# fraunhoferhhi/vvenc

Hardware: AMD Instinct MI355X
Metric: frames/sec + bit-exact vs CPU, 1080p/4K 10-bit preset=faster at 1/2/4/8 GPU (higher is better)
Workload: dtype i16; 1 GPU; BASELINE configs[1]: hot-path work lists RECORDED from the reference encoder (1920x1080 10-bit synthetic clip, 65 frames, preset faster; one picture per temporal layer), replayed resident in HBM: a step = one picture's integer-ME SAD windows + sub-pel SATD stages + table calls + fused TU transform/quant lists + DMVR lists on 5 HIP streams; steps follow the GOP's 1:1:2:4:8:16 layer mix from the key; hip_streams=5, sample_pairs_per_frame=175309451, coefficients_per_frame=6951461, recorded_calls_outside_the_lists=0

## Files before the change

vvenc_amd/csrc/me.hip:

```cpp
#include <stdlib.h>
#ifndef VVHIP_ME_HU
#define VVHIP_ME_HU 2
#endif
#ifndef VVHIP_ME_STAGE_WAVES
#define VVHIP_ME_STAGE_WAVES 6
#endif
#ifndef VVHIP_ME_ITEM_WAVES
#define VVHIP_ME_ITEM_WAVES 8
#endif
#include <string.h>
#include <algorithm>
#include <vector>
#include "common.h"
#include "hadtile.h"

struct vvhip_me_plan
{
  int bitDepth = 0, nCands = 0, nStages = 0, nItems = 0, nMaskItems = 0, maxPlane = 0;
  int wavesInt = 0, wavesStage = 0, wavesItem = 0, wavesItemMain = 0, ldsInt = 0, ldsStage = 0;
  int intBig = 0, ldsIntSmall = 0;
  int intLarge = 0, ldsIntMid = 0;
  bool stageAtomic = false;
  bool intSplit = false;
  bool timing = false; hipEvent_t ev[5] = { nullptr, nullptr, nullptr, nullptr, nullptr };
// ... 148 lines not shown
  { 0, 64, 0, 0 }, { -1, 63, 2, 0 }, { -2, 62, 4, 0 }, { -2, 60, 7, -1 }, { -2, 58, 10, -2 }, { -3, 57, 12, -2 }, { -4, 56, 14, -2 }, { -4, 55, 15, -2 }, { -4, 54, 16, -2 },
  { -5, 53, 18, -2 }, { -6, 52, 20, -2 }, { -6, 49, 24, -3 }, { -6, 46, 28, -4 }, { -5, 44, 29, -4 }, { -4, 42, 30, -4 }, { -4, 39, 33, -4 }, { -4, 36, 36, -4 } };

static int stageTap( int frac, int k, int filterMode, int altHpel )
{
  if( altHpel && frac == 8 ) return kAltHpel[k];
  if( filterMode == 2 )
  {
    const int ph = frac << 1;
    return ( k < 2 || k > 5 ) ? 0 : ( ph <= 16 ? kChroma4[ph][k - 2] : kChroma4[32 - ph][5 - k] );
  }
  const int p = frac <= 8 ? frac : 16 - frac, kk = frac <= 8 ? k : 7 - k;
  return filterMode == 0 ? kLuma8[p][kk] : kLuma6[p][kk];
}

static std::vector<int32_t> stageTapTables( int bitDepth )
{
  const int headRoom = 14 - bitDepth > 2 ? 14 - bitDepth : 2, vScale = 1 << ( 10 - headRoom ), hScale = 1 << ( 2 + headRoom );
  std::vector<int32_t> tapTab( 6 * 192, 0 );
  for( int mode = 0; mode < 3; mode++ ) for( int alt = 0; alt < 2; alt++ )
  {
    int32_t* t = &tapTab[( mode * 2 + alt ) * 192];
    const int set = ( mode == 2 && !alt ) ? 0 : ( mode == 0 ? 2 : 1 ), k0 = set == 0 ? 2 : ( set == 1 ? 1 : 0 ), np = set == 0 ? 2 : ( set == 1 ? 3 : 4 );
    for( int f = 0; f < 16; f++ )
    {
      for( int k = 0; k < 8; k++ ) t[f * 8 + k] = stageTap( f, k, mode, alt ) * vScale;
      for( int i = 0; i < 4; i++ ) t[128 + f * 4 + i] = i < np ? ( int32_t ) ( ( ( uint32_t ) ( stageTap( f, k0 + 2 * i, mode, alt ) * hScale ) & 0xffffu ) | ( ( uint32_t ) ( stageTap( f, k0 + 2 * i + 1, mode, alt ) * hScale ) << 16 ) ) : 0;
    }
  }
  return tapTab;
}

__device__ __forceinline__ void stagePos( const vvhip_me_stage_job& j, int k, int& tx, int& ty )
{
  constexpr uint32_t RX  = 1u | 1u << 2 | 1u << 4 | 0u << 6 | 2u << 8 | 0u << 10 | 2u << 12 | 0u << 14 | 2u << 16;
  constexpr uint32_t RYH = 1u | 0u << 2 | 2u << 4 | 1u << 6 | 1u << 8 | 0u << 10 | 0u << 12 | 2u << 14 | 2u << 16;
  constexpr uint32_t RYQ = 1u | 0u << 2 | 2u << 4 | 0u << 6 | 0u << 8 | 1u << 10 | 1u << 12 | 2u << 14 | 2u << 16;
  const int rx = ( int ) ( ( RX >> ( 2 * k ) ) & 3u ) - 1, ry = ( int ) ( ( ( j.i_frac == 2 ? RYH : RYQ ) >> ( 2 * k ) ) & 3u ) - 1;
  tx = ( rx + j.base_qx ) * j.i_frac * 4; ty = ( ry + j.base_qy ) * j.i_frac * 4;
}

template<int NT> struct VTaps { int c[NT]; };
template<int K0, int K1>
__device__ __forceinline__ void loadVTaps( const int* tapL, int fyk, VTaps<K1 - K0 + 1>& vt )
{
#pragma unroll
  for( int t = 0; t < K1 - K0 + 1; t++ ) vt.c[t] = tapL[fyk * 8 + K0 + t];
}
__device__ __forceinline__ int madLo( uint32_t v, int c, int acc ) { int r; asm( "v_mad_i32_i16 %0, %1, %2, %3" : "=v"( r ) : "v"( v ), "v"( c ), "v"( acc ) ); return r; }
__device__ __forceinline__ int madHi( uint32_t v, int c, int acc ) { int r; asm( "v_mad_i32_i16 %0, %1, %2, %3 op_sel:[1,0,0,0]" : "=v"( r ) : "v"( v ), "v"( c ), "v"( acc ) ); return r; }
__device__ __forceinline__ int mulLo( uint32_t v, int c ) { int r; asm( "v_mad_i32_i16 %0, %1, %2, 0" : "=v"( r ) : "v"( v ), "v"( c ) ); return r; }
__device__ __forceinline__ int med3( int v, int hi ) { int r; asm( "v_med3_i32 %0, %1, 0, %2" : "=v"( r ) : "v"( v ), "v"( hi ) ); return r; }
__device__ __forceinline__ int mulHi( uint32_t v, int c ) { int r; asm( "v_mad_i32_i16 %0, %1, %2, 0 op_sel:[1,0,0,0]" : "=v"( r ) : "v"( v ), "v"( c ) ); return r; }
template<int K0, int K1>
__device__ __forceinline__ void predRow( const int16_t* tv , int w, int y, int syk, bool anyFrac,
                                         const VTaps<K1 - K0 + 1>& vt, int headRoom, uint32_t maxPk, uint32_t ( &o )[4] )
{
  constexpr int NT = K1 - K0 + 1;
  if( anyFrac )
  {
    int acc[8];
#pragma unroll
    for( int t = 0; t < NT; t++ )
    {
      const int c = vt.c[t];
      const u32x4 r = *reinterpret_cast<const u32x4*>( tv + __mul24( y + syk + t + 1, w ) );
      if( t == 0 )
      {
        acc[0] = mulLo( r.x, c ); acc[1] = mulHi( r.x, c ); acc[2] = mulLo( r.y, c ); acc[3] = mulHi( r.y, c );
        acc[4] = mulLo( r.z, c ); acc[5] = mulHi( r.z, c ); acc[6] = mulLo( r.w, c ); acc[7] = mulHi( r.w, c );
      }
      else
      {
        acc[0] = madLo( r.x, c, acc[0] ); acc[1] = madHi( r.x, c, acc[1] ); acc[2] = madLo( r.y, c, acc[2] ); acc[3] = madHi( r.y, c, acc[3] );
        acc[4] = madLo( r.z, c, acc[4] ); acc[5] = madHi( r.z, c, acc[5] ); acc[6] = madLo( r.w, c, acc[6] ); acc[7] = madHi( r.w, c, acc[7] );
      }
    }
    const int maxS = ( int ) ( ( ( maxPk & 0xffffu ) << 16 ) | 0xffffu );
#pragma unroll
    for( int i = 0; i < 8; i++ ) acc[i] = med3( acc[i], maxS );
#pragma unroll
    for( int i = 0; i < 4; i++ ) o[i] = __builtin_amdgcn_perm( ( uint32_t ) acc[2 * i + 1], ( uint32_t ) acc[2 * i], 0x07060302u );
  }
  else
  {
    const u32x4 r = *reinterpret_cast<const u32x4*>( tv + __mul24( y + syk + 4 - K0, w ) );
    const uint32_t rw[4] = { r.x, r.y, r.z, r.w };
    const s16x2 sh = { ( short ) headRoom, ( short ) headRoom }, z = { 0, 0 };
#pragma unroll
    for( int i = 0; i < 4; i++ )
      o[i] = __builtin_bit_cast( uint32_t, __builtin_elementwise_min( __builtin_elementwise_max( __builtin_bit_cast( s16x2, rw[i] ) >> sh, z ), __builtin_bit_cast( s16x2, maxPk ) ) );
  }
}

__device__ __forceinline__ void avgInts( const uint32_t ( &ra )[4], const uint32_t ( &rb )[4], int ( &o )[4] )
{
#pragma unroll
  for( int i = 0; i < 4; i++ ) o[i] = dot2( pkAdd( ra[i], rb[i] ), 0x00010001u, 2 ) >> 2;
}

__device__ __forceinline__ int dot2s( uint32_t a, uint32_t b, int c ) { int r; asm( "v_dot2_i32_i16 %0, %1, %2, %3" : "=v"( r ) : "v"( a ), "v"( b ), "s"( c ) ); return r; }

template<int K0, int K1, bool ONE>
__device__ __forceinline__ void firstPass( const char* refB, int rs, int nH, int G, int log2G, int rowsT, int ldsPitch, int v0, int hx0, int hx1, int hx2,
                                           const uint32_t* tapP, int16_t* tmp, int tid, int offS, int headRoom, uint32_t biasPk )
{
  constexpr int NT = K1 - K0 + 1, NP = NT / 2, B0 = ( NT - 2 ) / 2, HU = VVHIP_ME_HU;
  const int txOne = v0 == 0 ? hx0 : ( v0 == 1 ? hx1 : hx2 );
  for( int ub = tid; ub < nH; ub += HU * 64 )
  {
    u32x4 LA[HU], LB[HU]; int fxs[HU], at[HU]; bool ok[HU];
#pragma unroll
    for( int q = 0; q < HU; q++ )
    {
      const int u = ub + q * 64;
      ok[q] = u < nH;
      const int uu = ok[q] ? u : ub;
      const int x0 = ( uu & ( G - 1 ) ) << 3, rr = uu >> log2G;
      int r = rr, txv = txOne;
      if( !ONE )
      {
        const int vl = ( rr >= rowsT ) + ( rr >= 2 * rowsT ), v = v0 + vl;
        r = rr - __mul24( vl, rowsT ); txv = v == 0 ? hx0 : ( v == 1 ? hx1 : hx2 );
      }
      fxs[q] = txv & 15; at[q] = __mul24( rr, ldsPitch ) + x0;
      const uint32_t off = ( uint32_t ) ( __mul24( r, rs ) + x0 + ( txv >> 4 ) + 8 ) * 2u;
      LA[q] = ld16o( refB, fxs[q] ? off + ( uint32_t ) ( 2 * ( K0 - 3 ) ) : off );
      if( fxs[q] ) LB[q] = ld16o( refB, off + ( uint32_t ) ( 2 * ( K0 - 3 + NT - 1 ) ) );
    }
#pragma unroll
    for( int q = 0; q < HU; q++ )
    {
      if( !ok[q] ) continue;
      const int fxv = fxs[q];
      const u32x4 A = LA[q];
      u32x4 ov;
      if( fxv )
      {
        const u32x4 B = LB[q];
        uint32_t W[4 + NP], S[4 + NP];
        W[0] = A.x; W[1] = A.y; W[2] = A.z; W[3] = A.w;
        S[B0] = B.x; S[B0 + 1] = B.y; S[B0 + 2] = B.z; S[B0 + 3] = B.w;
#pragma unroll
        for( int m = B0 - 1; m >= 0; m-- ) S[m] = __builtin_amdgcn_alignbit( W[m + 1], W[m], 16 );
#pragma unroll
        for( int m = 4; m < 4 + NP - 1; m++ ) W[m] = __builtin_amdgcn_alignbit( S[m], S[m - 1], 16 );
        uint32_t cp[NP];
#pragma unroll
        for( int i = 0; i < NP; i++ ) cp[i] = tapP[fxv * 4 + i];
        uint32_t o[4];
#pragma unroll
        for( int qq = 0; qq < 4; qq++ )
        {
          int e = dot2s( W[qq], cp[0], offS ), d = dot2s( S[qq], cp[0], offS );
#pragma unroll
          for( int i = 1; i < NP; i++ ) { e = dot2( W[qq + i], cp[i], e ); d = dot2( S[qq + i], cp[i], d ); }
          o[qq] = __builtin_amdgcn_perm( ( uint32_t ) d, ( uint32_t ) e, 0x06050201u );
        }
        ov.x = o[0]; ov.y = o[1]; ov.z = o[2]; ov.w = o[3];
      }
      else
      {
        const uint32_t aw[4] = { A.x, A.y, A.z, A.w };
        const s16x2 sh = { ( short ) headRoom, ( short ) headRoom };
        uint32_t o[4];
#pragma unroll
        for( int qq = 0; qq < 4; qq++ ) o[qq] = pkAdd( __builtin_bit_cast( uint32_t, __builtin_bit_cast( s16x2, aw[qq] ) << sh ), biasPk );
        ov.x = o[0]; ov.y = o[1]; ov.z = o[2]; ov.w = o[3];
      }
      *reinterpret_cast<u32x4*>( tmp + at[q] ) = ov;
    }
  }
}

constexpr int ST_STAGE_MASK = 0x3fffff, ST_VAR_SHIFT = 22;
constexpr int ST_UNIT_CONT = 1 << 28, ST_UNIT_MORE = 1 << 29, ST_UNIT_ATOMIC = 1 << 30;

template<int K0, int K1, bool GEN>
__device__ __forceinline__ void stageBody( const MePlanes& P, const MeArgs& a, const WaveSpan span, int16_t* lds, uint32_t* pairCost, const int wv )
{
  constexpr int NT = K1 - K0 + 1;
#define ST_SYNC() { __builtin_amdgcn_fence( __ATOMIC_ACQ_REL, "wavefront" ); __builtin_amdgcn_wave_barrier(); }
  const int tid = threadIdx.x & 63, nthr = 64, lane = tid, bd = a.bitDepth;
  const int headRoom = 14 - bd > 2 ? 14 - bd : 2;
  const int offS = ( 1 << ( headRoom - 1 ) ) << 8;
  const uint32_t biasPk = ( uint32_t ) ( 1 << ( headRoom - 1 ) ) * 0x00010001u;
  const uint32_t maxPk = ( uint32_t ) ( ( 1 << bd ) - 1 ) * 0x00010001u;
  int* tapL = reinterpret_cast<int*>( lds );
  uint32_t* tapP = reinterpret_cast<uint32_t*>( lds ) + 128;
  int* posL = reinterpret_cast<int*>( lds ) + 128 + 64;
  uint32_t* costL = reinterpret_cast<uint32_t*>( lds ) + 128 + 64 + 16;
  int16_t* tmp = lds + 2 * ( 128 + 64 + 16 + 16 );

  int curTab = -1;
  if( K0 == 2 )
  {
    for( int i = tid; i < 192; i += nthr ) reinterpret_cast<int*>( lds )[i] = a.tapTables[4 * 192 + i];
    curTab = 4;
  }
  for( int si = 0; si < span.count; si++ )
  {
    const StageUnit* up = a.stageUnits + span.first + si;
    const vvhip_me_stage_job j = up->j;
    const int unit = up->order, stage = unit & ST_STAGE_MASK, varOnly = ( unit >> ST_VAR_SHIFT ) & 3;
    const int w = j.width, h = j.height, uw = w < 64 ? w : 64, uwH = uw < 8 ? 8 : uw, G = uwH >> 3, log2G = 31 - __builtin_clz( G );
    const int BH = h < 32 ? h : 32, rowsT = BH + NT, y0 = ( ( unit >> 24 ) & 7 ) * BH, xoff = ( ( unit >> 27 ) & 1 ) * 64;
    const int ldsPitch = uwH + 8;
    const int rs = P.stride[j.ref_plane];
    const char* refB = reinterpret_cast<const char*>( P.p[j.ref_plane] + j.ref_off + xoff + ( ptrdiff_t ) ( y0 + K0 - 4 ) * rs - 8 );
    const char* orgB = reinterpret_cast<const char*>( P.p[j.org_plane] + j.org_off + xoff );
    const int os = P.stride[j.org_plane] ? P.stride[j.org_plane] : w;
    const int hx0 = up->hx[0], hx1 = up->hx[1], hx2 = up->hx[2], nHor = up->nHor, nPos = up->nPos, cnt0 = up->cnt0, cnt1 = up->cnt1;
    const int myPos = tid < 9 ? up->pos[tid] : 0;
    ST_SYNC();
    if( tid < 9 ) posL[tid] = myPos;
    const int tabId = j.filter_mode * 2 + ( j.alt_hpel ? 1 : 0 );
    if( tabId != curTab )
    {
      for( int i = tid; i < 192; i += nthr ) reinterpret_cast<int*>( lds )[i] = a.tapTables[tabId * 192 + i];
      curTab = tabId;
    }
    if( !( unit & ST_UNIT_CONT ) && tid < 9 ) costL[tid] = 0;
    const int kind = j.func == VVHIP_DF_SAD ? TK_ROWS : ( GEN ? hadTileKind( w, h, j.func == VVHIP_DF_HAD_FAST ) : ( ( j.func == VVHIP_DF_HAD_FAST && ( w & 31 ) == 0 ) ? TK_16F : TK_8x8 ) );
    const bool rows4 = GEN && ( kind == TK_4x8 || ( kind == TK_ROWS && uw == 4 ) );
    const int log2PW = !GEN ? ( kind == TK_16F ? 4 : 3 ) : ( rows4 ? 2 : ( kind == TK_ROWS ? 3 : 31 - __builtin_clz( tileW( kind ) ) ) );
    const int log2PH = !GEN ? ( kind == TK_16F ? 4 : 3 ) : ( rows4 ? 3 : ( kind == TK_ROWS ? ( BH < 8 ? 31 - __builtin_clz( BH ) : 3 ) : 31 - __builtin_clz( tileH( kind ) ) ) );
    const int log2LT = !GEN ? 3 : ( rows4 ? 2 : ( kind == TK_ROWS ? log2PH : 31 - __builtin_clz( tileLanes( kind ) ) ) ), LT = 1 << log2LT;
    const int log2TX = ( 31 - __builtin_clz( uw ) ) - log2PW, log2TB = log2TX + ( 31 - __builtin_clz( BH ) ) - log2PH, tilesX = 1 << log2TX;
    const int vpp = uw <= 16 ? nHor : 1;
    for( int v0 = varOnly ? varOnly - 1 : 0; v0 < ( varOnly ? varOnly : nHor ); v0 += vpp )
    {
    const int nV = nHor - v0 < vpp ? nHor - v0 : vpp;
    const int pBeg = v0 == 0 ? 0 : ( v0 == 1 ? cnt0 : cnt0 + cnt1 ), pEnd = v0 + nV >= 3 ? nPos : ( v0 + nV == 2 ? cnt0 + cnt1 : ( v0 + nV == 1 ? cnt0 : 0 ) );
    ST_SYNC();
#if defined( VVHIP_ME_CUT ) && ( VVHIP_ME_CUT & 1 )
    const int nH = 0;
#else
    const int nH = nV * rowsT * G;
#endif
    if( nV == 1 ) firstPass<K0, K1, true>( refB, rs, nH, G, log2G, rowsT, ldsPitch, v0, hx0, hx1, hx2, tapP, tmp, tid, offS, headRoom, biasPk );
    else          firstPass<K0, K1, false>( refB, rs, nH, G, log2G, rowsT, ldsPitch, v0, hx0, hx1, hx2, tapP, tmp, tid, offS, headRoom, biasPk );
    ST_SYNC();     
#if defined( VVHIP_ME_CUT ) && ( VVHIP_ME_CUT & 2 )
    const int nPP = 0;
#else
    const int nPP = pEnd - pBeg;
#endif
    const int log2L = log2TB + log2LT, log2Lw = log2L < 6 ? log2L : 6;
    const int trips = log2L > 6 ? 1 << ( log2L - 6 ) : 1, PL = 64 >> log2Lw, plLane = tid >> log2Lw;
    for( int c = 0; c < trips && nPP > 0; c++ )
    {
      const int sl = ( c << 6 ) + ( tid & ( ( 1 << log2Lw ) - 1 ) ), r = sl & ( LT - 1 ), t = sl >> log2LT;
      const int tyi = t >> log2TX, txi = t & ( tilesX - 1 );
      uint32_t o4[4] = { 0, 0, 0, 0 };
      if( kind == TK_16F )
      {
// ... 10 lines not shown
        o4[0] = oa.x; o4[1] = oa.y; o4[2] = ob.x; o4[3] = ob.y;
      }
      else
      {
        const int row = ( GEN && kind == TK_16x8 ) ? tyi * 8 + ( r & 7 ) : ( tyi << log2PH ) + r, col = ( GEN && kind == TK_16x8 ) ? txi * 16 + 8 * ( r >> 3 ) : txi * 8;
        const u32x4 ovv = ld16o( orgB, ( uint32_t ) ( __mul24( y0 + row, os ) + col ) * 2u );
        o4[0] = ovv.x; o4[1] = ovv.y; o4[2] = ovv.z; o4[3] = ovv.w;
      }
      for( int p0 = 0; p0 < nPP; p0 += PL )
      {
      const int pl = p0 + plLane;
      const bool valid = pl < nPP;
      const int pi = pBeg + ( valid ? pl : 0 );
      const int pk = posL[pi], txk = ( ( pk >> 8 ) & 0xfff ) - 64, tyk = ( ( pk >> 20 ) & 0xfff ) - 64;
      const int hv = ( txk == hx0 ? 0 : ( ( nHor > 1 && txk == hx1 ) ? 1 : 2 ) ) - v0, syk = tyk >> 4, fyk = tyk & 15;
      const int16_t* tvp = tmp + hv * rowsT * ldsPitch;
      const bool anyFrac = __builtin_amdgcn_ballot_w64( fyk != 0 ) != 0;
      VTaps<NT> vt;
      if( anyFrac ) loadVTaps<K0, K1>( tapL, fyk, vt );
      uint32_t sres;
      if( kind == TK_16F )
      {
        uint32_t D[4];
        const int16_t* tv = tvp + txi * 16;
        uint32_t pa[4], pb[4]; int ap[4];
        predRow<K0, K1>( tv, ldsPitch, tyi * 16 + 2 * r, syk, anyFrac, vt, headRoom, maxPk, pa );
        predRow<K0, K1>( tv, ldsPitch, tyi * 16 + 2 * r + 1, syk, anyFrac, vt, headRoom, maxPk, pb );
        avgInts( pa, pb, ap );
        D[0] = pkSub( o4[0], pkInts( ap[0], ap[1] ) ); D[1] = pkSub( o4[1], pkInts( ap[2], ap[3] ) );
        predRow<K0, K1>( tv + 8, ldsPitch, tyi * 16 + 2 * r, syk, anyFrac, vt, headRoom, maxPk, pa );
        predRow<K0, K1>( tv + 8, ldsPitch, tyi * 16 + 2 * r + 1, syk, anyFrac, vt, headRoom, maxPk, pb );
        avgInts( pa, pb, ap );
        D[2] = pkSub( o4[2], pkInts( ap[0], ap[1] ) ); D[3] = pkSub( o4[3], pkInts( ap[2], ap[3] ) );
        sres = hadTeamPkD( D, r, GEN ? LT : 8, TK_16F, lane );
      }
      else
      {
        uint32_t p4[4];
        if( rows4 )
        {
          const int row = tyi * 8 + 2 * r;
          uint32_t pa[4], pb[4];
          predRow<K0, K1>( tvp, ldsPitch, row, syk, anyFrac, vt, headRoom, maxPk, pa );
          predRow<K0, K1>( tvp, ldsPitch, row + 1, syk, anyFrac, vt, headRoom, maxPk, pb );
          p4[0] = pa[0]; p4[1] = pa[1]; p4[2] = pb[0]; p4[3] = pb[1];
        }
        else
        {
          const int row = ( GEN && kind == TK_16x8 ) ? tyi * 8 + ( r & 7 ) : ( tyi << log2PH ) + r, col = ( GEN && kind == TK_16x8 ) ? txi * 16 + 8 * ( r >> 3 ) : txi * 8;
          predRow<K0, K1>( tvp + col, ldsPitch, row, syk, anyFrac, vt, headRoom, maxPk, p4 );
        }
        if( kind == TK_ROWS )
        {
          uint32_t sa = 0;
#pragma unroll
          for( int i = 0; i < 4; i++ ) sa = __builtin_amdgcn_sad_u16( o4[i] ^ BIAS, p4[i] ^ BIAS, sa );
          sres = vvhipGroupSum32( sa, LT, lane );
        }
        else sres = hadTeamPk( o4, p4, r, GEN ? LT : 8, GEN ? kind : TK_8x8, lane );
      }
      if( valid && r == 0 ) atomicAdd( &costL[pk & 0xff], sres );
      }
    }
    }
    ST_SYNC();     
    if( unit & ST_UNIT_MORE ) continue;
    if( GEN && ( unit & ST_UNIT_ATOMIC ) )
    {
      if( tid < 9 && ( ( j.mask >> tid ) & 1 ) ) atomicAdd( reinterpret_cast<unsigned long long*>( a.stageCost ) + ( size_t ) 9 * stage + tid, ( unsigned long long ) costL[tid] );
    }
    else
    {
      const int ownBeg = varOnly <= 1 ? 0 : ( varOnly == 2 ? cnt0 : cnt0 + cnt1 ), ownEnd = !varOnly ? nPos : ( varOnly == 1 ? cnt0 : ( varOnly == 2 ? cnt0 + cnt1 : nPos ) );
      const bool pair = !( h <= 32 && w <= 64 );
      if( pair ) { if( wv == 1 && tid < 9 ) pairCost[tid] = costL[tid]; __syncthreads(); }
      if( !pair || wv == 0 )
      {
        if( !varOnly ) { if( tid < 9 ) a.stageCost[( size_t ) 9 * stage + tid] = ( ( j.mask >> tid ) & 1 ) ? costL[tid] + ( pair ? pairCost[tid] : 0u ) : 0u; }
        else
        {
          if( tid >= ownBeg && tid < ownEnd ) { const int k = posL[tid] & 0xff; a.stageCost[( size_t ) 9 * stage + k] = costL[k] + ( pair ? pairCost[k] : 0u ); }
          if( varOnly == 1 && tid < 9 && !( ( j.mask >> tid ) & 1 ) ) a.stageCost[( size_t ) 9 * stage + tid] = 0u;
        }
      }
      if( pair ) __syncthreads();
    }
  }
}

__device__ __forceinline__ uint32_t ld4( const int16_t* p ) { struct __attribute__( ( packed, aligned( 2 ) ) ) U4 { uint32_t v; }; return ( ( const ME_GLOBAL U4* ) p )->v; }

__device__ __forceinline__ void maskItemBody( const MeArgs& a, const WaveSpan span, int nItems, const int16_t* const* planeL, const int* strideL, int lane )
{
  const int first = span.first, count = -span.count;
  const vvhip_me_mask_item f = a.maskItems[first];
  const int w = f.width, h = f.height, ss = f.sub_shift;
  const int cw = w >= 8 ? 8 : ( w >= 4 ? 4 : 2 ), lprShift = ( 31 - __builtin_clz( w ) ) - ( 31 - __builtin_clz( cw ) ), lpr = 1 << lprShift, rowsEff = h >> ss, chunks = rowsEff * lpr;
// ... 266 lines not shown

int hostWinPitch( int winW ) { return 2 * ( ( ( winW + 3 ) >> 1 ) | 1 ); }
int hostWinSamples( int winW, int winH ) { return ( winH * hostWinPitch( winW ) + 7 ) & ~7; }

}

#ifndef VVHIP_ME_KERNELS_ONLY
extern "C" {

static int mePlanCreate( vvhip_ctx* ctx, const vvhip_me_lists& L, int bit_depth, int max_window, vvhip_me_plan** out );

int vvhip_get_me_tap_tables_host( int bit_depth, int32_t* host_out )
{
  if( bit_depth < 8 || bit_depth > 10 || !host_out ) return VVHIP_E_ARG;
  const std::vector<int32_t> t = stageTapTables( bit_depth );
  memcpy( host_out, t.data(), t.size() * sizeof( int32_t ) );
  return VVHIP_OK;
}

int vvhip_me_plan_create( vvhip_ctx* ctx, const vvhip_me_int_job* int_jobs, int n_int_jobs, const vvhip_me_cand* cands, int n_cands,
                          const vvhip_me_stage_job* stage_jobs, int n_stage_jobs, const vvhip_me_item* items, int n_items, int bit_depth, int max_window, vvhip_me_plan** out )
{
  vvhip_me_lists L; L.int_jobs = int_jobs; L.n_int_jobs = n_int_jobs; L.cands = cands; L.n_cands = n_cands; L.stage_jobs = stage_jobs; L.n_stage_jobs = n_stage_jobs;
  L.items = items; L.n_items = n_items; L.mask_items = nullptr; L.n_mask_items = 0;
  return mePlanCreate( ctx, L, bit_depth, max_window, out );
}

int vvhip_me_plan_create_lists( vvhip_ctx* ctx, const vvhip_me_lists* lists, int bit_depth, int max_window, vvhip_me_plan** out )
{
  if( !ctx || !lists ) return VVHIP_E_ARG;
  return mePlanCreate( ctx, *lists, bit_depth, max_window, out );
// ... 162 lines not shown
    int count = 0, work = 0;
    if( dealOf( s0 ) == 0 ) count = unitsOf( s0 ) / 2;
    else if( dealOf( s0 ) == 1 ) count = 1;
    else
      while( i + count < stOrder.size() && count < 8 )
      {
        const vvhip_me_stage_job& s = stage_jobs[stOrder[i + count] & ST_STAGE_MASK];
        if( unitW( s ) != unitW( s0 ) || setOf( s ) != setOf( s0 ) || dealOf( s ) != 2 || ( count && work + unitWork( s ) > bundleWork ) ) break;
        work += unitWork( s ); count++;
      }
    WaveSpan sp; sp.first = ( int32_t ) i; sp.count = count; stWaves.push_back( sp );
    setWaves[setOf( s0 )]++;
    int bh = unitH( s0 );
    for( int u = 1; u < count; u++ ) bh = std::max( bh, unitH( stage_jobs[stOrder[i + u] & ST_STAGE_MASK] ) );
    const int nt = tapSetOf( s0 ) == 0 ? 4 : ( tapSetOf( s0 ) == 1 ? 6 : 8 ), uw = std::max( 8, unitW( s0 ) ), vpp = unitW( s0 ) <= 16 ? 3 : 1;
    const int ldsUnit = ( 2 * ( 128 + 64 + 16 + 16 ) + vpp * ( bh + nt ) * ( uw + 8 ) ) * 2;
    setLds[setOf( s0 )] = std::max( setLds[setOf( s0 )], ( ldsUnit + 15 ) & ~15 );
    ldsStage = std::max( ldsStage, ldsUnit );
    i += count;
  }

  if( band )
  {
    std::vector<WaveSpan> src( stWaves );
    for( int k = 0, first = 0; k < 6; first += setWaves[k], k++ )
    {
      auto subOf = [&]( int w ) { const vvhip_me_stage_job& s = stage_jobs[stOrder[src[first + w].first] & ST_STAGE_MASK]; return ( 2 - dealOf( s ) ) * 1024 + unitW( s ); };
      for( int w0 = 0; w0 < setWaves[k]; )
      {
        int w1 = w0;
        while( w1 < setWaves[k] && subOf( w1 ) == subOf( w0 ) ) w1++;
// ... 305 lines not shown
```

Measured before the change: 15150 frames/s.

## Interleave row pairs in LDS for dot2 vertical sub-pel filtering

The horizontal first pass now writes two source rows interleaved per 32-bit word in LDS, with pitch counted in dwords. The vertical filter then uses packed v_dot2_i32_i16 with odd/even paired tap tables instead of per-row 16-bit multiply-adds. The 16-wide tile path computes both rows of a pair from a single set of loads. The aim is to cut vertical-filter instruction count and LDS reads, at the cost of larger tap tables, extra permute work on integer-position rows, and the removal of the HU unroll knob.

```diff
diff --git a/vvenc_amd/csrc/me.hip b/vvenc_amd/csrc/me.hip
--- a/vvenc_amd/csrc/me.hip
+++ b/vvenc_amd/csrc/me.hip
@@ -1,7 +1,4 @@
 #include <stdlib.h>
-#ifndef VVHIP_ME_HU
-#define VVHIP_ME_HU 2
-#endif
 #ifndef VVHIP_ME_STAGE_WAVES
 #define VVHIP_ME_STAGE_WAVES 6
 #endif
@@ -186,18 +183,25 @@
   return filterMode == 0 ? kLuma8[p][kk] : kLuma6[p][kk];
 }
 
+constexpr int TAP_TAB = 352;
 static std::vector<int32_t> stageTapTables( int bitDepth )
 {
   const int headRoom = 14 - bitDepth > 2 ? 14 - bitDepth : 2, vScale = 1 << ( 10 - headRoom ), hScale = 1 << ( 2 + headRoom );
-  std::vector<int32_t> tapTab( 6 * 192, 0 );
+  std::vector<int32_t> tapTab( 6 * TAP_TAB, 0 );
   for( int mode = 0; mode < 3; mode++ ) for( int alt = 0; alt < 2; alt++ )
   {
-    int32_t* t = &tapTab[( mode * 2 + alt ) * 192];
-    const int set = ( mode == 2 && !alt ) ? 0 : ( mode == 0 ? 2 : 1 ), k0 = set == 0 ? 2 : ( set == 1 ? 1 : 0 ), np = set == 0 ? 2 : ( set == 1 ? 3 : 4 );
+    int32_t* t = &tapTab[( mode * 2 + alt ) * TAP_TAB];
+    const int set = ( mode == 2 && !alt ) ? 0 : ( mode == 0 ? 2 : 1 ), k0 = set == 0 ? 2 : ( set == 1 ? 1 : 0 ), np = set == 0 ? 2 : ( set == 1 ? 3 : 4 ), vps = np + 1;
     for( int f = 0; f < 16; f++ )
     {
       for( int k = 0; k < 8; k++ ) t[f * 8 + k] = stageTap( f, k, mode, alt ) * vScale;
       for( int i = 0; i < 4; i++ ) t[128 + f * 4 + i] = i < np ? ( int32_t ) ( ( ( uint32_t ) ( stageTap( f, k0 + 2 * i, mode, alt ) * hScale ) & 0xffffu ) | ( ( uint32_t ) ( stageTap( f, k0 + 2 * i + 1, mode, alt ) * hScale ) << 16 ) ) : 0;
+      auto c = [&]( int i ) { return ( i < 0 || i >= 2 * np ) ? 0u : ( uint32_t ) ( stageTap( f, k0 + i, mode, alt ) * vScale ) & 0xffffu; };
+      for( int i = 0; i < vps; i++ )
+      {
+        t[192 + f * 2 * vps + i]       = ( int32_t ) ( c( 2 * i - 1 ) | ( c( 2 * i ) << 16 ) );
+        t[192 + f * 2 * vps + vps + i] = ( int32_t ) ( c( 2 * i ) | ( c( 2 * i + 1 ) << 16 ) );
+      }
     }
   }
   return tapTab;
@@ -212,138 +216,219 @@
   tx = ( rx + j.base_qx ) * j.i_frac * 4; ty = ( ry + j.base_qy ) * j.i_frac * 4;
 }
 
-template<int NT> struct VTaps { int c[NT]; };
+template<int NT> struct VTaps { uint32_t o[NT / 2 + 1], e[NT / 2]; };
 template<int K0, int K1>
-__device__ __forceinline__ void loadVTaps( const int* tapL, int fyk, VTaps<K1 - K0 + 1>& vt )
-{
-#pragma unroll
-  for( int t = 0; t < K1 - K0 + 1; t++ ) vt.c[t] = tapL[fyk * 8 + K0 + t];
-}
-__device__ __forceinline__ int madLo( uint32_t v, int c, int acc ) { int r; asm( "v_mad_i32_i16 %0, %1, %2, %3" : "=v"( r ) : "v"( v ), "v"( c ), "v"( acc ) ); return r; }
-__device__ __forceinline__ int madHi( uint32_t v, int c, int acc ) { int r; asm( "v_mad_i32_i16 %0, %1, %2, %3 op_sel:[1,0,0,0]" : "=v"( r ) : "v"( v ), "v"( c ), "v"( acc ) ); return r; }
-__device__ __forceinline__ int mulLo( uint32_t v, int c ) { int r; asm( "v_mad_i32_i16 %0, %1, %2, 0" : "=v"( r ) : "v"( v ), "v"( c ) ); return r; }
+__device__ __forceinline__ void loadVTaps( const uint32_t* tapV, int fyk, VTaps<K1 - K0 + 1>& vt )
+{
+  constexpr int VPS = ( K1 - K0 + 1 ) / 2 + 1;
+#pragma unroll
+  for( int t = 0; t < VPS; t++ ) { vt.o[t] = tapV[fyk * 2 * VPS + t]; if( t < VPS - 1 ) vt.e[t] = tapV[fyk * 2 * VPS + VPS + t]; }
+}
+__device__ __forceinline__ int dot2z( uint32_t a, uint32_t b ) { int r; asm( "v_dot2_i32_i16 %0, %1, %2, 0" : "=v"( r ) : "v"( a ), "v"( b ) ); return r; }
 __device__ __forceinline__ int med3( int v, int hi ) { int r; asm( "v_med3_i32 %0, %1, 0, %2" : "=v"( r ) : "v"( v ), "v"( hi ) ); return r; }
-__device__ __forceinline__ int mulHi( uint32_t v, int c ) { int r; asm( "v_mad_i32_i16 %0, %1, %2, 0 op_sel:[1,0,0,0]" : "=v"( r ) : "v"( v ), "v"( c ) ); return r; }
+__device__ __forceinline__ void avgInts( const uint32_t ( &ra )[4], const uint32_t ( &rb )[4], int ( &o )[4] )
+{
+#pragma unroll
+  for( int i = 0; i < 4; i++ ) o[i] = dot2( pkAdd( ra[i], rb[i] ), 0x00010001u, 2 ) >> 2;
+}
+__device__ __forceinline__ void clipPack8( int ( &acc )[8], uint32_t maxPk, uint32_t ( &o )[4] )
+{
+  const int maxS = ( int ) ( ( ( maxPk & 0xffffu ) << 16 ) | 0xffffu );
+#pragma unroll
+  for( int i = 0; i < 8; i++ ) acc[i] = med3( acc[i], maxS );
+#pragma unroll
+  for( int i = 0; i < 4; i++ ) o[i] = __builtin_amdgcn_perm( ( uint32_t ) acc[2 * i + 1], ( uint32_t ) acc[2 * i], 0x07060302u );
+}
+__device__ __forceinline__ void copyClip4( const uint32_t ( &rw )[4], int headRoom, uint32_t maxPk, uint32_t ( &o )[4] )
+{
+  const s16x2 sh = { ( short ) headRoom, ( short ) headRoom }, z = { 0, 0 };
+#pragma unroll
+  for( int i = 0; i < 4; i++ )
+    o[i] = __builtin_bit_cast( uint32_t, __builtin_elementwise_min( __builtin_elementwise_max( __builtin_bit_cast( s16x2, rw[i] ) >> sh, z ), __builtin_bit_cast( s16x2, maxPk ) ) );
+}
 template<int K0, int K1>
-__device__ __forceinline__ void predRow( const int16_t* tv , int w, int y, int syk, bool anyFrac,
+__device__ __forceinline__ void predRow( const uint32_t* tv , int pitchD, int y, int syk, bool anyFrac,
                                          const VTaps<K1 - K0 + 1>& vt, int headRoom, uint32_t maxPk, uint32_t ( &o )[4] )
 {
-  constexpr int NT = K1 - K0 + 1;
+  constexpr int NT = K1 - K0 + 1, VPS = NT / 2 + 1;
   if( anyFrac )
   {
+    const int a = y + syk + 1;
+    const bool odd = a & 1;
+    const uint32_t* p = tv + __mul24( a >> 1, pitchD );
     int acc[8];
 #pragma unroll
-    for( int t = 0; t < NT; t++ )
-    {
-      const int c = vt.c[t];
-      const u32x4 r = *reinterpret_cast<const u32x4*>( tv + __mul24( y + syk + t + 1, w ) );
-      if( t == 0 )
-      {
-        acc[0] = mulLo( r.x, c ); acc[1] = mulHi( r.x, c ); acc[2] = mulLo( r.y, c ); acc[3] = mulHi( r.y, c );
-        acc[4] = mulLo( r.z, c ); acc[5] = mulHi( r.z, c ); acc[6] = mulLo( r.w, c ); acc[7] = mulHi( r.w, c );
-      }
-      else
-      {
-        acc[0] = madLo( r.x, c, acc[0] ); acc[1] = madHi( r.x, c, acc[1] ); acc[2] = madLo( r.y, c, acc[2] ); acc[3] = madHi( r.y, c, acc[3] );
-        acc[4] = madLo( r.z, c, acc[4] ); acc[5] = madHi( r.z, c, acc[5] ); acc[6] = madLo( r.w, c, acc[6] ); acc[7] = madHi( r.w, c, acc[7] );
-      }
-    }
+    for( int i = 0; i < VPS; i++ )
+    {
+      const uint32_t c = odd ? vt.o[i] : ( i < VPS - 1 ? vt.e[i] : 0u );
+      const u32x4 r0 = *reinterpret_cast<const u32x4*>( p + i * pitchD ), r1 = *reinterpret_cast<const u32x4*>( p + i * pitchD + 4 );
+      const uint32_t d[8] = { r0.x, r0.y, r0.z, r0.w, r1.x, r1.y, r1.z, r1.w };
+#pragma unroll
+      for( int x = 0; x < 8; x++ ) acc[x] = i == 0 ? dot2z( d[x], c ) : dot2( d[x], c, acc[x] );
+    }
+    clipPack8( acc, maxPk, o );
+  }
+  else
+  {
+    const int R = y + syk + 4 - K0;
+    const uint32_t* p = tv + __mul24( R >> 1, pitchD );
+    const uint32_t hb = ( uint32_t ) ( R & 1 ) << 1, sel = 0x05040100u + __builtin_amdgcn_perm( hb, hb, 0u );
+    const u32x4 r0 = *reinterpret_cast<const u32x4*>( p ), r1 = *reinterpret_cast<const u32x4*>( p + 4 );
+    const uint32_t rw[4] = { __builtin_amdgcn_perm( r0.y, r0.x, sel ), __builtin_amdgcn_perm( r0.w, r0.z, sel ), __builtin_amdgcn_perm( r1.y, r1.x, sel ), __builtin_amdgcn_perm( r1.w, r1.z, sel ) };
+    copyClip4( rw, headRoom, maxPk, o );
+  }
+}
+template<int K0, int K1, int E>
+__device__ __forceinline__ void pred16F( const uint32_t* tv, int pitchD, int y, int syk, bool anyFrac, const VTaps<K1 - K0 + 1>& vt, int headRoom, uint32_t maxPk,
+                                         uint32_t ( &po )[4], uint32_t ( &pe )[4] )
+{
+  constexpr int NT = K1 - K0 + 1, NP = NT / 2, VPS = NP + 1;
+  if( anyFrac )
+  {
+    const int a = y + syk + 1;
+    const uint32_t* p = tv + __mul24( a >> 1, pitchD );
     const int maxS = ( int ) ( ( ( maxPk & 0xffffu ) << 16 ) | 0xffffu );
 #pragma unroll
-    for( int i = 0; i < 8; i++ ) acc[i] = med3( acc[i], maxS );
-#pragma unroll
-    for( int i = 0; i < 4; i++ ) o[i] = __builtin_amdgcn_perm( ( uint32_t ) acc[2 * i + 1], ( uint32_t ) acc[2 * i], 0x07060302u );
+    for( int hf = 0; hf < 2; hf++ )
+    {
+      int accO[4], accE[4];
+#pragma unroll
+      for( int i = 0; i < VPS; i++ )
+      {
+        const u32x4 rr = *reinterpret_cast<const u32x4*>( p + i * pitchD + hf * 4 );
+        const uint32_t d[4] = { rr.x, rr.y, rr.z, rr.w };
+        const int ie = i - E;
+#pragma unroll
+        for( int x = 0; x < 4; x++ )
+        {
+          accO[x] = i == 0 ? dot2z( d[x], vt.o[i] ) : dot2( d[x], vt.o[i], accO[x] );
+          if( ie >= 0 && ie < NP ) accE[x] = ie == 0 ? dot2z( d[x], vt.e[ie] ) : dot2( d[x], vt.e[ie], accE[x] );
+        }
+      }
+#pragma unroll
+      for( int x = 0; x < 4; x++ ) { accO[x] = med3( accO[x], maxS ); accE[x] = med3( accE[x], maxS ); }
+#pragma unroll
+      for( int x = 0; x < 2; x++ )
+      {
+        po[hf * 2 + x] = __builtin_amdgcn_perm( ( uint32_t ) accO[2 * x + 1], ( uint32_t ) accO[2 * x], 0x07060302u );
+        pe[hf * 2 + x] = __builtin_amdgcn_perm( ( uint32_t ) accE[2 * x + 1], ( uint32_t ) accE[2 * x], 0x07060302u );
+      }
+    }
+  }
+  else if( ( ( E + 3 - K0 ) & 1 ) == 0 )
+  {
+    const uint32_t* p = tv + __mul24( ( y + syk + 4 - K0 ) >> 1, pitchD );
+    const u32x4 r0 = *reinterpret_cast<const u32x4*>( p ), r1 = *reinterpret_cast<const u32x4*>( p + 4 );
+    const uint32_t lo[4] = { __builtin_amdgcn_perm( r0.y, r0.x, 0x05040100u ), __builtin_amdgcn_perm( r0.w, r0.z, 0x05040100u ), __builtin_amdgcn_perm( r1.y, r1.x, 0x05040100u ), __builtin_amdgcn_perm( r1.w, r1.z, 0x05040100u ) };
+    const uint32_t hi[4] = { __builtin_amdgcn_perm( r0.y, r0.x, 0x07060302u ), __builtin_amdgcn_perm( r0.w, r0.z, 0x07060302u ), __builtin_amdgcn_perm( r1.y, r1.x, 0x07060302u ), __builtin_amdgcn_perm( r1.w, r1.z, 0x07060302u ) };
+    copyClip4( lo, headRoom, maxPk, po );
+    copyClip4( hi, headRoom, maxPk, pe );
   }
   else
   {
-    const u32x4 r = *reinterpret_cast<const u32x4*>( tv + __mul24( y + syk + 4 - K0, w ) );
-    const uint32_t rw[4] = { r.x, r.y, r.z, r.w };
-    const s16x2 sh = { ( short ) headRoom, ( short ) headRoom }, z = { 0, 0 };
-#pragma unroll
-    for( int i = 0; i < 4; i++ )
-      o[i] = __builtin_bit_cast( uint32_t, __builtin_elementwise_min( __builtin_elementwise_max( __builtin_bit_cast( s16x2, rw[i] ) >> sh, z ), __builtin_bit_cast( s16x2, maxPk ) ) );
-  }
-}
-
-__device__ __forceinline__ void avgInts( const uint32_t ( &ra )[4], const uint32_t ( &rb )[4], int ( &o )[4] )
-{
-#pragma unroll
-  for( int i = 0; i < 4; i++ ) o[i] = dot2( pkAdd( ra[i], rb[i] ), 0x00010001u, 2 ) >> 2;
+    const uint32_t* p = tv + __mul24( ( y + syk + 4 - K0 ) >> 1, pitchD );
+    const u32x4 r0 = *reinterpret_cast<const u32x4*>( p ), r1 = *reinterpret_cast<const u32x4*>( p + 4 );
+    const u32x4 q0 = *reinterpret_cast<const u32x4*>( p + pitchD ), q1 = *reinterpret_cast<const u32x4*>( p + pitchD + 4 );
+    const uint32_t hi[4] = { __builtin_amdgcn_perm( r0.y, r0.x, 0x07060302u ), __builtin_amdgcn_perm( r0.w, r0.z, 0x07060302u ), __builtin_amdgcn_perm( r1.y, r1.x, 0x07060302u ), __builtin_amdgcn_perm( r1.w, r1.z, 0x07060302u ) };
+    const uint32_t lo[4] = { __builtin_amdgcn_perm( q0.y, q0.x, 0x05040100u ), __builtin_amdgcn_perm( q0.w, q0.z, 0x05040100u ), __builtin_amdgcn_perm( q1.y, q1.x, 0x05040100u ), __builtin_amdgcn_perm( q1.w, q1.z, 0x05040100u ) };
+    copyClip4( hi, headRoom, maxPk, po );
+    copyClip4( lo, headRoom, maxPk, pe );
+  }
+}
+template<int K0, int K1, int E>
+__device__ __forceinline__ void tile16F( const uint32_t* tv, int pitchD, int y, int syk, bool anyFrac, const VTaps<K1 - K0 + 1>& vt, int headRoom, uint32_t maxPk,
+                                         const uint32_t ( &o4 )[4], uint32_t ( &D )[4] )
+{
+#pragma unroll
+  for( int hc = 0; hc < 2; hc++ )
+  {
+    uint32_t pa[4], pb[4]; int ap[4];
+    pred16F<K0, K1, E>( tv + hc * 8, pitchD, y, syk, anyFrac, vt, headRoom, maxPk, pa, pb );
+    avgInts( pa, pb, ap );
+    D[2 * hc] = pkSub( o4[2 * hc], pkInts( ap[0], ap[1] ) ); D[2 * hc + 1] = pkSub( o4[2 * hc + 1], pkInts( ap[2], ap[3] ) );
+  }
 }
 
 __device__ __forceinline__ int dot2s( uint32_t a, uint32_t b, int c ) { int r; asm( "v_dot2_i32_i16 %0, %1, %2, %3" : "=v"( r ) : "v"( a ), "v"( b ), "s"( c ) ); return r; }
 
 template<int K0, int K1, bool ONE>
-__device__ __forceinline__ void firstPass( const char* refB, int rs, int nH, int G, int log2G, int rowsT, int ldsPitch, int v0, int hx0, int hx1, int hx2,
-                                           const uint32_t* tapP, int16_t* tmp, int tid, int offS, int headRoom, uint32_t biasPk )
-{
-  constexpr int NT = K1 - K0 + 1, NP = NT / 2, B0 = ( NT - 2 ) / 2, HU = VVHIP_ME_HU;
-  const int txOne = v0 == 0 ? hx0 : ( v0 == 1 ? hx1 : hx2 );
-  for( int ub = tid; ub < nH; ub += HU * 64 )
-  {
-    u32x4 LA[HU], LB[HU]; int fxs[HU], at[HU]; bool ok[HU];
-#pragma unroll
-    for( int q = 0; q < HU; q++ )
-    {
-      const int u = ub + q * 64;
-      ok[q] = u < nH;
-      const int uu = ok[q] ? u : ub;
-      const int x0 = ( uu & ( G - 1 ) ) << 3, rr = uu >> log2G;
-      int r = rr, txv = txOne;
-      if( !ONE )
-      {
-        const int vl = ( rr >= rowsT ) + ( rr >= 2 * rowsT ), v = v0 + vl;
-        r = rr - __mul24( vl, rowsT ); txv = v == 0 ? hx0 : ( v == 1 ? hx1 : hx2 );
-      }
-      fxs[q] = txv & 15; at[q] = __mul24( rr, ldsPitch ) + x0;
-      const uint32_t off = ( uint32_t ) ( __mul24( r, rs ) + x0 + ( txv >> 4 ) + 8 ) * 2u;
-      LA[q] = ld16o( refB, fxs[q] ? off + ( uint32_t ) ( 2 * ( K0 - 3 ) ) : off );
-      if( fxs[q] ) LB[q] = ld16o( refB, off + ( uint32_t ) ( 2 * ( K0 - 3 + NT - 1 ) ) );
-    }
-#pragma unroll
-    for( int q = 0; q < HU; q++ )
-    {
-      if( !ok[q] ) continue;
-      const int fxv = fxs[q];
-      const u32x4 A = LA[q];
-      u32x4 ov;
-      if( fxv )
-      {
-        const u32x4 B = LB[q];
-        uint32_t W[4 + NP], S[4 + NP];
-        W[0] = A.x; W[1] = A.y; W[2] = A.z; W[3] = A.w;
-        S[B0] = B.x; S[B0 + 1] = B.y; S[B0 + 2] = B.z; S[B0 + 3] = B.w;
-#pragma unroll
-        for( int m = B0 - 1; m >= 0; m-- ) S[m] = __builtin_amdgcn_alignbit( W[m + 1], W[m], 16 );
-#pragma unroll
-        for( int m = 4; m < 4 + NP - 1; m++ ) W[m] = __builtin_amdgcn_alignbit( S[m], S[m - 1], 16 );
-        uint32_t cp[NP];
-#pragma unroll
-        for( int i = 0; i < NP; i++ ) cp[i] = tapP[fxv * 4 + i];
-        uint32_t o[4];
-#pragma unroll
-        for( int qq = 0; qq < 4; qq++ )
+__device__ __forceinline__ void firstPass( const char* refB, int rs, int nHP, int G, int log2G, int rowsT, int pitchD, int v0, int hx0, int hx1, int hx2,
+                                           const uint32_t* tapP, uint32_t* tmp, int tid, int offS, int headRoom, uint32_t biasPk )
+{
+  constexpr int NT = K1 - K0 + 1, NP = NT / 2, B0 = ( NT - 2 ) / 2;
+  const int txOne = v0 == 0 ? hx0 : ( v0 == 1 ? hx1 : hx2 ), pairsT = rowsT >> 1;
+  for( int u = tid; u < nHP; u += 64 )
+  {
+    const int x0 = ( u & ( G - 1 ) ) << 3, pp = u >> log2G;
+    int pr = pp, txv = txOne;
+    if( !ONE )
+    {
+      const int vl = ( pp >= pairsT ) + ( pp >= 2 * pairsT ), v = v0 + vl;
+      pr = pp - __mul24( vl, pairsT ); txv = v == 0 ? hx0 : ( v == 1 ? hx1 : hx2 );
+    }
+    const int fxv = txv & 15;
+    uint32_t* const dst = tmp + __mul24( pp, pitchD ) + x0;
+    const uint32_t off = ( uint32_t ) ( __mul24( 2 * pr, rs ) + x0 + ( txv >> 4 ) + 8 ) * 2u;
+    u32x4 LA[2], LB[2];
+#pragma unroll
+    for( int q = 0; q < 2; q++ )
+    {
+      const uint32_t offq = off + ( uint32_t ) q * ( uint32_t ) rs * 2u;
+      LA[q] = ld16o( refB, fxv ? offq + ( uint32_t ) ( 2 * ( K0 - 3 ) ) : offq );
+      if( fxv ) LB[q] = ld16o( refB, offq + ( uint32_t ) ( 2 * ( K0 - 3 + NT - 1 ) ) );
+    }
+    uint32_t ov[8];
+    if( fxv )
+    {
+      uint32_t cp[NP];
+#pragma unroll
+      for( int i = 0; i < NP; i++ ) cp[i] = tapP[fxv * 4 + i];
+      uint32_t W[2][4 + NP], S[2][4 + NP];
+#pragma unroll
+      for( int q = 0; q < 2; q++ )
+      {
+        const u32x4 A = LA[q], B = LB[q];
+        W[q][0] = A.x; W[q][1] = A.y; W[q][2] = A.z; W[q][3] = A.w;
+        S[q][B0] = B.x; S[q][B0 + 1] = B.y; S[q][B0 + 2] = B.z; S[q][B0 + 3] = B.w;
+#pragma unroll
+        for( int m = B0 - 1; m >= 0; m-- ) S[q][m] = __builtin_amdgcn_alignbit( W[q][m + 1], W[q][m], 16 );
+#pragma unroll
+        for( int m = 4; m < 4 + NP - 1; m++ ) W[q][m] = __builtin_amdgcn_alignbit( S[q][m], S[q][m - 1], 16 );
+      }
+#pragma unroll
+      for( int qq = 0; qq < 4; qq++ )
+      {
+        int e[2], d[2];
+#pragma unroll
+        for( int q = 0; q < 2; q++ )
         {
-          int e = dot2s( W[qq], cp[0], offS ), d = dot2s( S[qq], cp[0], offS );
-#pragma unroll
-          for( int i = 1; i < NP; i++ ) { e = dot2( W[qq + i], cp[i], e ); d = dot2( S[qq + i], cp[i], d ); }
-          o[qq] = __builtin_amdgcn_perm( ( uint32_t ) d, ( uint32_t ) e, 0x06050201u );
+          e[q] = dot2s( W[q][qq], cp[0], offS ); d[q] = dot2s( S[q][qq], cp[0], offS );
+#pragma unroll
+          for( int i = 1; i < NP; i++ ) { e[q] = dot2( W[q][qq + i], cp[i], e[q] ); d[q] = dot2( S[q][qq + i], cp[i], d[q] ); }
         }
-        ov.x = o[0]; ov.y = o[1]; ov.z = o[2]; ov.w = o[3];
-      }
-      else
-      {
-        const uint32_t aw[4] = { A.x, A.y, A.z, A.w };
-        const s16x2 sh = { ( short ) headRoom, ( short ) headRoom };
-        uint32_t o[4];
-#pragma unroll
-        for( int qq = 0; qq < 4; qq++ ) o[qq] = pkAdd( __builtin_bit_cast( uint32_t, __builtin_bit_cast( s16x2, aw[qq] ) << sh ), biasPk );
-        ov.x = o[0]; ov.y = o[1]; ov.z = o[2]; ov.w = o[3];
-      }
-      *reinterpret_cast<u32x4*>( tmp + at[q] ) = ov;
-    }
-  }
-}
+        ov[2 * qq]     = __builtin_amdgcn_perm( ( uint32_t ) e[1], ( uint32_t ) e[0], 0x06050201u );
+        ov[2 * qq + 1] = __builtin_amdgcn_perm( ( uint32_t ) d[1], ( uint32_t ) d[0], 0x06050201u );
+      }
+    }
+    else
+    {
+      const uint32_t aw[2][4] = { { LA[0].x, LA[0].y, LA[0].z, LA[0].w }, { LA[1].x, LA[1].y, LA[1].z, LA[1].w } };
+      const s16x2 sh = { ( short ) headRoom, ( short ) headRoom };
+#pragma unroll
+      for( int qq = 0; qq < 4; qq++ )
+      {
+        const uint32_t ra = pkAdd( __builtin_bit_cast( uint32_t, __builtin_bit_cast( s16x2, aw[0][qq] ) << sh ), biasPk );
+        const uint32_t rb = pkAdd( __builtin_bit_cast( uint32_t, __builtin_bit_cast( s16x2, aw[1][qq] ) << sh ), biasPk );
+        ov[2 * qq] = __builtin_amdgcn_perm( rb, ra, 0x05040100u ); ov[2 * qq + 1] = __builtin_amdgcn_perm( rb, ra, 0x07060302u );
+      }
+    }
+    u32x4 s0, s1;
+    s0.x = ov[0]; s0.y = ov[1]; s0.z = ov[2]; s0.w = ov[3]; s1.x = ov[4]; s1.y = ov[5]; s1.z = ov[6]; s1.w = ov[7];
+    *reinterpret_cast<u32x4*>( dst ) = s0; *reinterpret_cast<u32x4*>( dst + 4 ) = s1;
+  }
+}
+
+__device__ __forceinline__ bool maskBit( uint32_t mask, int k ) { return __builtin_amdgcn_ubfe( mask, ( uint32_t ) k, 1u ) != 0; }
 
 constexpr int ST_STAGE_MASK = 0x3fffff, ST_VAR_SHIFT = 22;
 constexpr int ST_UNIT_CONT = 1 << 28, ST_UNIT_MORE = 1 << 29, ST_UNIT_ATOMIC = 1 << 30;
@@ -358,16 +443,17 @@
   const int offS = ( 1 << ( headRoom - 1 ) ) << 8;
   const uint32_t biasPk = ( uint32_t ) ( 1 << ( headRoom - 1 ) ) * 0x00010001u;
   const uint32_t maxPk = ( uint32_t ) ( ( 1 << bd ) - 1 ) * 0x00010001u;
-  int* tapL = reinterpret_cast<int*>( lds );
-  uint32_t* tapP = reinterpret_cast<uint32_t*>( lds ) + 128;
-  int* posL = reinterpret_cast<int*>( lds ) + 128 + 64;
-  uint32_t* costL = reinterpret_cast<uint32_t*>( lds ) + 128 + 64 + 16;
-  int16_t* tmp = lds + 2 * ( 128 + 64 + 16 + 16 );
+  constexpr int VPS = NT / 2 + 1, TABW = 64 + 32 * VPS;
+  uint32_t* tapP = reinterpret_cast<uint32_t*>( lds );
+  uint32_t* tapV = reinterpret_cast<uint32_t*>( lds ) + 64;
+  int* posL = reinterpret_cast<int*>( lds ) + TABW;
+  uint32_t* costL = reinterpret_cast<uint32_t*>( lds ) + TABW + 12;
+  uint32_t* tmp = reinterpret_cast<uint32_t*>( lds ) + TABW + 24;
 
   int curTab = -1;
   if( K0 == 2 )
   {
-    for( int i = tid; i < 192; i += nthr ) reinterpret_cast<int*>( lds )[i] = a.tapTables[4 * 192 + i];
+    for( int i = tid; i < TABW; i += nthr ) reinterpret_cast<int*>( lds )[i] = a.tapTables[4 * TAP_TAB + 128 + i];
     curTab = 4;
   }
   for( int si = 0; si < span.count; si++ )
@@ -377,7 +463,7 @@
     const int unit = up->order, stage = unit & ST_STAGE_MASK, varOnly = ( unit >> ST_VAR_SHIFT ) & 3;
     const int w = j.width, h = j.height, uw = w < 64 ? w : 64, uwH = uw < 8 ? 8 : uw, G = uwH >> 3, log2G = 31 - __builtin_clz( G );
     const int BH = h < 32 ? h : 32, rowsT = BH + NT, y0 = ( ( unit >> 24 ) & 7 ) * BH, xoff = ( ( unit >> 27 ) & 1 ) * 64;
-    const int ldsPitch = uwH + 8;
+    const int pitchD = uwH + 4;
     const int rs = P.stride[j.ref_plane];
     const char* refB = reinterpret_cast<const char*>( P.p[j.ref_plane] + j.ref_off + xoff + ( ptrdiff_t ) ( y0 + K0 - 4 ) * rs - 8 );
     const char* orgB = reinterpret_cast<const char*>( P.p[j.org_plane] + j.org_off + xoff );
@@ -389,7 +475,7 @@
     const int tabId = j.filter_mode * 2 + ( j.alt_hpel ? 1 : 0 );
     if( tabId != curTab )
     {
-      for( int i = tid; i < 192; i += nthr ) reinterpret_cast<int*>( lds )[i] = a.tapTables[tabId * 192 + i];
+      for( int i = tid; i < TABW; i += nthr ) reinterpret_cast<int*>( lds )[i] = a.tapTables[tabId * TAP_TAB + 128 + i];
       curTab = tabId;
     }
     if( !( unit & ST_UNIT_CONT ) && tid < 9 ) costL[tid] = 0;
@@ -406,12 +492,12 @@
     const int pBeg = v0 == 0 ? 0 : ( v0 == 1 ? cnt0 : cnt0 + cnt1 ), pEnd = v0 + nV >= 3 ? nPos : ( v0 + nV == 2 ? cnt0 + cnt1 : ( v0 + nV == 1 ? cnt0 : 0 ) );
     ST_SYNC();
 #if defined( VVHIP_ME_CUT ) && ( VVHIP_ME_CUT & 1 )
-    const int nH = 0;
+    const int nHP = 0;
 #else
-    const int nH = nV * rowsT * G;
+    const int nHP = nV * ( rowsT >> 1 ) * G;
 #endif
-    if( nV == 1 ) firstPass<K0, K1, true>( refB, rs, nH, G, log2G, rowsT, ldsPitch, v0, hx0, hx1, hx2, tapP, tmp, tid, offS, headRoom, biasPk );
-    else          firstPass<K0, K1, false>( refB, rs, nH, G, log2G, rowsT, ldsPitch, v0, hx0, hx1, hx2, tapP, tmp, tid, offS, headRoom, biasPk );
+    if( nV == 1 ) firstPass<K0, K1, true>( refB, rs, nHP, G, log2G, rowsT, pitchD, v0, hx0, hx1, hx2, tapP, tmp, tid, offS, headRoom, biasPk );
+    else          firstPass<K0, K1, false>( refB, rs, nHP, G, log2G, rowsT, pitchD, v0, hx0, hx1, hx2, tapP, tmp, tid, offS, headRoom, biasPk );
     ST_SYNC();     
 #if defined( VVHIP_ME_CUT ) && ( VVHIP_ME_CUT & 2 )
     const int nPP = 0;
@@ -452,24 +538,17 @@
       const int pi = pBeg + ( valid ? pl : 0 );
       const int pk = posL[pi], txk = ( ( pk >> 8 ) & 0xfff ) - 64, tyk = ( ( pk >> 20 ) & 0xfff ) - 64;
       const int hv = ( txk == hx0 ? 0 : ( ( nHor > 1 && txk == hx1 ) ? 1 : 2 ) ) - v0, syk = tyk >> 4, fyk = tyk & 15;
-      const int16_t* tvp = tmp + hv * rowsT * ldsPitch;
+      const uint32_t* tvp = tmp + hv * ( rowsT >> 1 ) * pitchD;
       const bool anyFrac = __builtin_amdgcn_ballot_w64( fyk != 0 ) != 0;
       VTaps<NT> vt;
-      if( anyFrac ) loadVTaps<K0, K1>( tapL, fyk, vt );
+      if( anyFrac ) loadVTaps<K0, K1>( tapV, fyk, vt );
       uint32_t sres;
       if( kind == TK_16F )
       {
         uint32_t D[4];
-        const int16_t* tv = tvp + txi * 16;
-        uint32_t pa[4], pb[4]; int ap[4];
-        predRow<K0, K1>( tv, ldsPitch, tyi * 16 + 2 * r, syk, anyFrac, vt, headRoom, maxPk, pa );
-        predRow<K0, K1>( tv, ldsPitch, tyi * 16 + 2 * r + 1, syk, anyFrac, vt, headRoom, maxPk, pb );
-        avgInts( pa, pb, ap );
-        D[0] = pkSub( o4[0], pkInts( ap[0], ap[1] ) ); D[1] = pkSub( o4[1], pkInts( ap[2], ap[3] ) );
-        predRow<K0, K1>( tv + 8, ldsPitch, tyi * 16 + 2 * r, syk, anyFrac, vt, headRoom, maxPk, pa );
-        predRow<K0, K1>( tv + 8, ldsPitch, tyi * 16 + 2 * r + 1, syk, anyFrac, vt, headRoom, maxPk, pb );
-        avgInts( pa, pb, ap );
-        D[2] = pkSub( o4[2], pkInts( ap[0], ap[1] ) ); D[3] = pkSub( o4[3], pkInts( ap[2], ap[3] ) );
+        const uint32_t* tv = tvp + txi * 16;
+        if( syk & 1 ) tile16F<K0, K1, 0>( tv, pitchD, tyi * 16 + 2 * r, syk, anyFrac, vt, headRoom, maxPk, o4, D );
+        else          tile16F<K0, K1, 1>( tv, pitchD, tyi * 16 + 2 * r, syk, anyFrac, vt, headRoom, maxPk, o4, D );
         sres = hadTeamPkD( D, r, GEN ? LT : 8, TK_16F, lane );
       }
       else
@@ -479,14 +558,14 @@
         {
           const int row = tyi * 8 + 2 * r;
           uint32_t pa[4], pb[4];
-          predRow<K0, K1>( tvp, ldsPitch, row, syk, anyFrac, vt, headRoom, maxPk, pa );
-          predRow<K0, K1>( tvp, ldsPitch, row + 1, syk, anyFrac, vt, headRoom, maxPk, pb );
+          predRow<K0, K1>( tvp, pitchD, row, syk, anyFrac, vt, headRoom, maxPk, pa );
+          predRow<K0, K1>( tvp, pitchD, row + 1, syk, anyFrac, vt, headRoom, maxPk, pb );
           p4[0] = pa[0]; p4[1] = pa[1]; p4[2] = pb[0]; p4[3] = pb[1];
         }
         else
         {
           const int row = ( GEN && kind == TK_16x8 ) ? tyi * 8 + ( r & 7 ) : ( tyi << log2PH ) + r, col = ( GEN && kind == TK_16x8 ) ? txi * 16 + 8 * ( r >> 3 ) : txi * 8;
-          predRow<K0, K1>( tvp + col, ldsPitch, row, syk, anyFrac, vt, headRoom, maxPk, p4 );
+          predRow<K0, K1>( tvp + col, pitchD, row, syk, anyFrac, vt, headRoom, maxPk, p4 );
         }
         if( kind == TK_ROWS )
         {
@@ -505,7 +584,7 @@
     if( unit & ST_UNIT_MORE ) continue;
     if( GEN && ( unit & ST_UNIT_ATOMIC ) )
     {
-      if( tid < 9 && ( ( j.mask >> tid ) & 1 ) ) atomicAdd( reinterpret_cast<unsigned long long*>( a.stageCost ) + ( size_t ) 9 * stage + tid, ( unsigned long long ) costL[tid] );
+      if( tid < 9 && maskBit( j.mask, tid ) ) atomicAdd( reinterpret_cast<unsigned long long*>( a.stageCost ) + ( size_t ) ( 9 * stage + tid ), ( unsigned long long ) costL[tid] );
     }
     else
     {
@@ -514,11 +593,11 @@
       if( pair ) { if( wv == 1 && tid < 9 ) pairCost[tid] = costL[tid]; __syncthreads(); }
       if( !pair || wv == 0 )
       {
-        if( !varOnly ) { if( tid < 9 ) a.stageCost[( size_t ) 9 * stage + tid] = ( ( j.mask >> tid ) & 1 ) ? costL[tid] + ( pair ? pairCost[tid] : 0u ) : 0u; }
+        if( !varOnly ) { if( tid < 9 ) a.stageCost[( size_t ) ( 9 * stage + tid )] = maskBit( j.mask, tid ) ? costL[tid] + ( pair ? pairCost[tid] : 0u ) : 0u; }
         else
         {
           if( tid >= ownBeg && tid < ownEnd ) { const int k = posL[tid] & 0xff; a.stageCost[( size_t ) 9 * stage + k] = costL[k] + ( pair ? pairCost[k] : 0u ); }
-          if( varOnly == 1 && tid < 9 && !( ( j.mask >> tid ) & 1 ) ) a.stageCost[( size_t ) 9 * stage + tid] = 0u;
+          if( varOnly == 1 && tid < 9 && !maskBit( j.mask, tid ) ) a.stageCost[( size_t ) ( 9 * stage + tid )] = 0u;
         }
       }
       if( pair ) __syncthreads();
@@ -815,7 +894,7 @@
 {
   if( bit_depth < 8 || bit_depth > 10 || !host_out ) return VVHIP_E_ARG;
   const std::vector<int32_t> t = stageTapTables( bit_depth );
-  memcpy( host_out, t.data(), t.size() * sizeof( int32_t ) );
+  for( int i = 0; i < 6; i++ ) memcpy( host_out + i * 192, t.data() + i * TAP_TAB, 192 * sizeof( int32_t ) );
   return VVHIP_OK;
 }
 
@@ -1008,7 +1087,7 @@
     int bh = unitH( s0 );
     for( int u = 1; u < count; u++ ) bh = std::max( bh, unitH( stage_jobs[stOrder[i + u] & ST_STAGE_MASK] ) );
     const int nt = tapSetOf( s0 ) == 0 ? 4 : ( tapSetOf( s0 ) == 1 ? 6 : 8 ), uw = std::max( 8, unitW( s0 ) ), vpp = unitW( s0 ) <= 16 ? 3 : 1;
-    const int ldsUnit = ( 2 * ( 128 + 64 + 16 + 16 ) + vpp * ( bh + nt ) * ( uw + 8 ) ) * 2;
+    const int ldsUnit = ( 2 * ( 64 + 32 * ( nt / 2 + 1 ) + 24 ) + vpp * ( bh + nt ) * ( uw + 4 ) ) * 2;
     setLds[setOf( s0 )] = std::max( setLds[setOf( s0 )], ( ldsUnit + 15 ) & ~15 );
     ldsStage = std::max( ldsStage, ldsUnit );
     i += count;
```

Result: no change. 15220 frames/s, median of 6 (+0.5%).
